# jweyn/DLWP-CS

Hardware: AMD Instinct MI355X
Metric: cubed-sphere samples/sec (fwd+bwd) (higher is better)
Workload: dtype bf16; 1 GPU; unet2 C48: x (32,6,48,48,14) per GPU, 14 out channels, base 32, MSE + Adam, fwd+bwd+update, bf16 activations + bf16 MFMA, fp32 master weights / gradients / Adam; global_batch=32, parallelism=dp1, hip_graphs=True

## Files before the change

dlwp-cs_amd/DLWP/_native.py:

```python
import ctypes
import os
import threading

import numpy as np
import torch

_HERE = os.path.dirname(os.path.abspath(__file__))
_TAG = os.environ.get('DLWPCS_LIB_TAG', '')
LIB_PATH = os.path.join(os.path.dirname(_HERE), 'lib', 'libdlwpcs%s.so' % ('_' + _TAG if _TAG else ''))

F32 = 0
BF16 = 1
I16 = 2
MAP_RENORMALIZE = 1
MSE_TARGET_F32 = 0x100
MSE_OVERWRITE = 0x200
ADAM_ZERO_GRAD = 1
HEAD_DEFER_STAGE2 = 2
LOSS_MSE, LOSS_MAE, LOSS_ACC = 0, 1, 2
REG_NONE, REG_MSE, REG_MAE, REG_GLOBAL = 0, 1, 2, 3
NORM_ALL, NORM_VALID = 0, 1
E_UNSUPPORTED = -2
ACT_NONE = 0
ACT_LEAKY_CLIP = 1
# ... 321 lines not shown
    'dlwpcs_state_repack': (c_int, [c_void_p, c_void_p, c_void_p, c_int, c_size_t, c_int, c_int, c_int, c_int, c_void_p]),
    'dlwpcs_head_mse_scratch_bytes': (c_size_t, []),
    'dlwpcs_head_mse_tail': (c_int, [c_void_p, c_float, c_int, c_void_p, c_void_p, c_void_p]),
    'dlwpcs_loss_tail_run': (c_int, [c_void_p, c_void_p]),
    'dlwpcs_head_mse_step': (c_int, [c_void_p, c_void_p, c_void_p, c_void_p, c_void_p, c_void_p, c_float, c_void_p, c_void_p,
                                     c_void_p, c_int, c_void_p, c_void_p]),
    'dlwpcs_head_mse_step_masked': (c_int, [c_void_p, c_void_p, c_void_p, c_void_p, c_void_p, c_void_p, c_float, c_void_p,
                                            c_void_p, c_void_p, c_int, c_void_p, c_float, c_float, c_void_p]),
    'dlwpcs_adam_step_dev': (c_int, [c_void_p, c_void_p, c_void_p, c_void_p, c_size_t, c_void_p, c_void_p, c_int,
                                     c_void_p]),
    'dlwpcs_batch_gather': (c_int, [c_void_p, ctypes.c_int64, c_int, ctypes.c_int64, c_void_p, c_int, c_void_p, c_int,
                                    c_int, c_int, c_int, c_void_p, c_int, c_int, c_int, c_int, c_int, c_void_p]),
    'dlwpcs_solar_fill': (c_int, [c_void_p, ctypes.c_int64, c_void_p, ctypes.c_int64, c_void_p, c_int, c_int, c_int, c_int,
                                  c_void_p, c_int, c_int, c_int, c_int, c_int, c_void_p]),
    'dlwpcs_channel_moments_scratch_bytes': (c_size_t, [c_void_p, ctypes.c_int64]),
    'dlwpcs_channel_moments': (c_int, [c_void_p, c_void_p, c_void_p, ctypes.c_int64, c_void_p, c_int, c_void_p, c_void_p, c_size_t,
                                       c_void_p]),
    'dlwpcs_channel_affine': (c_int, [c_void_p, c_void_p, c_void_p, c_void_p, c_int, c_void_p, c_void_p]),
    'dlwpcs_channel_range_scratch_bytes': (c_size_t, [ctypes.c_int64, ctypes.c_int64, ctypes.c_int64]),
    'dlwpcs_channel_range': (c_int, [c_void_p, ctypes.c_int64, ctypes.c_int64, ctypes.c_int64, c_void_p, c_void_p, c_void_p,
                                     c_size_t, c_void_p]),
    'dlwpcs_pack_i16': (c_int, [c_void_p, ctypes.c_int64, ctypes.c_int64, ctypes.c_int64, c_void_p, c_void_p, c_void_p, c_void_p]),
    'dlwpcs_unpack_i16': (c_int, [c_void_p, ctypes.c_int64, ctypes.c_int64, ctypes.c_int64, c_void_p, c_void_p, c_void_p,
                                  c_void_p]),
    'dlwpcs_batch_gather_i16': (c_int, [c_void_p, ctypes.c_int64, c_int, ctypes.c_int64, c_void_p, c_void_p, c_void_p, c_int,
                                        c_void_p, c_int, c_int, c_int, c_int, c_void_p, c_int, c_int, c_int, c_int, c_int,
                                        c_void_p]),
    'dlwpcs_comm_load': (c_int, [ctypes.c_char_p]),
    'dlwpcs_comm_unique_id': (c_int, [c_void_p]),
    'dlwpcs_comm_init': (c_int, [ctypes.POINTER(c_void_p), c_void_p, c_int, c_int]),
    'dlwpcs_comm_destroy': (c_int, [c_void_p]),
    'dlwpcs_allreduce_f32': (c_int, [c_void_p, c_void_p, c_size_t, c_void_p]),
    'dlwpcs_lds_oob_probe': (c_int, [c_void_p, c_void_p]),
    'dlwpcs_prof_enable': (c_int, [c_int]),
    'dlwpcs_prof_reset': (c_int, []),
    'dlwpcs_prof_count': (c_int, []),
    'dlwpcs_prof_get': (c_int, [c_int, ctypes.c_char_p, c_int, ctypes.POINTER(ctypes.c_double),
                                ctypes.POINTER(ctypes.c_double), ctypes.POINTER(ctypes.c_double)]),
    'dlwpcs_prof_known_tags': (c_int, []),
    'dlwpcs_prof_known_tag': (c_int, [c_int, ctypes.c_char_p, c_int]),
}

_lib = None
_lock = threading.Lock()


class NativeError(RuntimeError):
    pass


def lib():
    global _lib
    if _lib is None:
        with _lock:
            if _lib is None:
                if not os.path.exists(LIB_PATH):
                    raise NativeError(
                        'libdlwpcs.so not found at %s: build it with `python dlwp-cs_amd/build.py` '
                        '(or __graft_entry__.build()).  The DLWP-CS MI355X engine has no CPU fallback.' % LIB_PATH)
                handle = ctypes.CDLL(LIB_PATH)
                for name, (res, args) in PROTOTYPES.items():
                    fn = getattr(handle, name)
                    fn.restype = res
                    fn.argtypes = args
                _lib = handle
    return _lib
# ... 117 lines not shown
```

dlwp-cs_amd/csrc/conv_launch.h:

```cpp
#pragma once
#include "conv_ws.h"

namespace dlwpcs {

struct Work { double flops, bytes; };

static int tile_pixels(int BM, int No) {
    const int face_pix = No * No;
    int pix = BM < face_pix ? BM : face_pix;
    if (No <= BM) {
        int whole = (BM / No) * No;
        if (whole > face_pix) whole = face_pix;
        if (ceil_div(face_pix, whole) <= ceil_div(face_pix, pix)) pix = whole;
    }
    return pix;
}

static long ilv_cost(int pix, int face_pix, int B, int gx, int WM, int *gb, int *fb, bool split, int c2 = 2) {
    auto cost = [&](int npix) { const int mn = (npix + 31) / 32; return 4 * ceil_div(mn, WM) + c2; };
    const int nbl = ceil_div(face_pix, pix), cF = cost(pix), cL = cost(face_pix - (nbl - 1) * pix);
    const long ntiles = 6l * B * nbl;
    const long plain = (long)ceil_div((int)ntiles, gx) * cF;
    if (gb) *gb = 0;
    if (fb) *fb = 0;
    if (!split || cL >= cF || nbl < 2) return plain;
    const long F = 6l * (nbl - 1) * B, S = 6l * B;
    long best = plain;
    for (int GB = 1; GB < gx; ++GB) {
        const int GA = gx - GB;
        const long sB = ceil_div((int)S, GB) * (long)cL;
        for (long mB = 0; mB <= ceil_div((int)F, gx) + 1; ++mB) {
            const long FB = mB * GB < F ? mB * GB : F, FA = F - FB;
            const long cA = (long)ceil_div((int)FA, GA) * cF, cB = mB * cF + sB;
            const long mx = cA > cB ? cA : cB;
// ... 46 lines not shown
    P.magicNo = div_magic(P.No);
    P.magicN = div_magic(P.Nin);
    P.magicB = P.B > 1 ? div_magic(P.B) : 0;
    P.magicNblk = P.nblk_face > 1 ? div_magic(P.nblk_face) : 0;
    P.tile_rows_max = tile_rows_for(pix, P.Wt) + (KS - 1);
    P.ntiles = P.B * 6 * P.ncol * P.nblk_face;
    P.split_gb = P.split_fb = 0;
    P.tune = tune_bits();
    const size_t in_b = (size_t)P.tile_rows_max * P.W2 * (KC * ES + 16), w_b = (size_t)NTB * (KC / CGW) * (KS * KS + (EDGE ? 3 : 0)) * 1024;
    const bool rowpairs = (32 * MT) % (2 * P.Wt) == 0 && pix % (2 * P.Wt) == 0;
    const bool halfrows = !rowpairs && 32 * MT == P.Wt && WM == 4 && WN == 1 && pix == 4 * P.Wt && P.Wt % 4 == 0;
    bool pool = MODE != MODE_ZERO && P.pool_out != nullptr && P.No % 2 == 0 && P.Wt % 2 == 0 && (rowpairs || halfrows) &&
                strip_pix % pix == 0 && P.Cout % 32 == 0 && P.Cout % (16 / ES) == 0;
    if (EDGE) pool = pool && !MOUT && ES == 2 && P.dsplit > 0 && P.dsplit % 32 == 0;
    const size_t buf = in_b + w_b;
    size_t patch_b = (size_t)(WM * WN) * 32 * (32 * ES + 16);
    if (pool && 2 * buf + patch_b * MT <= 160 * 1024) patch_b *= MT; else pool = false;
    size_t lds = 2 * buf + patch_b;
    P.patches = 1;
    P.wstat = 0;
    const int nchunks = ceil_div(P.CG, KC / CGW);
    if (nchunks > 2 && nchunks <= 4 && (tune_bits() & TUNE_CONV_WSTAT) && 2 * in_b + nchunks * w_b + patch_b <= 160 * 1024) {
        P.wstat = nchunks;
        lds = 2 * in_b + nchunks * w_b + patch_b;
    } else if (lds > 160 * 1024) { lds = 2 * buf; P.patches = 0; pool = false; }
    if (!pool) P.pool_out = nullptr;
    {
        const bool head = P.head_w != nullptr && P.head_out != nullptr && ES == 2 && NT == 1 && WN == 1 && !EDGE && !MOUT && !MASK &&
                          MODE != MODE_ZERO && P.Cout == 32 && P.patches && !pool;
        if (head) P.out = P.head_out; else P.head_w = nullptr;
        if (P.head_done) *P.head_done = head ? 1 : 0;
    }
    P.colsplit = (pool && halfrows) ? 1 : 0;
    if (P.pool_done) *P.pool_done = pool ? 1 : 0;
    if ((MODE == MODE_ZERO || EDGE) && KS == 3 && P.patches && P.Cout % (16 / ES) == 0 && P.dsplit % (16 / ES) == 0) {
        if (P.direct_done) *P.direct_done = (P.d0 || P.d1) ? 1 : 0;
    } else {
        P.d0 = P.d1 = nullptr;
    }
    if (EDGE) {
        if (P.nblk_face < 2)
            return fail(DLWPCS_E_UNSUPPORTED, "conv: gather-form data gradient: a tile holds both edge rows of a face (N=%d)", P.No);
    }
    if (lds > 160 * 1024)
        return fail(DLWPCS_E_UNSUPPORTED, "conv: LDS tile of %zu bytes exceeds 160 KiB (face size %d)", lds, P.No);
    if (P.ncol > 1 && !P.patches)
        return fail(DLWPCS_E_UNSUPPORTED, "conv: internal: column strips need the line-store epilogue (face size %d)", P.No);
    if (P.tile_rows_max > 32)
        return fail(DLWPCS_E_UNSUPPORTED, "conv: %d tile rows exceed the producers' 5-bit row field", P.tile_rows_max);
    if ((size_t)P.tile_rows_max * P.W2 > (size_t)3 * NTHREADS)
        return fail(DLWPCS_E_UNSUPPORTED, "conv: tile of %d x %d pixels exceeds the producers' register capacity", P.tile_rows_max, P.W2);
    if ((long)6 * face_pix * P.Cout * ES >= (1l << 31))
        return fail(DLWPCS_E_UNSUPPORTED, "conv: one sample of the output (%ld bytes) exceeds the 32-bit store offsets",
                    (long)6 * face_pix * P.Cout * ES);
    if ((long)P.Nin * P.Nin * 6 >= (1l << 16) * 6 && (long)P.Nin * P.Nin >= (1l << 16))
        return fail(DLWPCS_E_UNSUPPORTED, "conv: face size %d too large for the 16-bit index arithmetic", P.Nin);
    auto kern = conv_mfma_ws_kernel<T, KS, KC, MT, NT, WM, WN, VW, MODE, MASK, TAIL8, MOUT, EDGE>;
    if (!MOUT || !(P.d0 || P.d1)) {
        if (!(P.d0)) P.m0 = nullptr;
        if (!(P.d1)) P.m1 = nullptr;
        if (!MOUT) P.m0 = P.m1 = nullptr;
    }
    if (P.mask_done) *P.mask_done = (MOUT && (P.m0 || P.m1)) ? ((P.m0 ? 1 : 0) | (P.m1 ? 2 : 0)) : 0;
    if (lds > 64 * 1024) {
        hipError_t e = hipFuncSetAttribute((const void *)kern, hipFuncAttributeMaxDynamicSharedMemorySize, (int)lds);
        if (e != hipSuccess) return fail(DLWPCS_E_LAUNCH, "conv: hipFuncSetAttribute: %s", hipGetErrorString(e));
// ... 64 lines not shown
```

dlwp-cs_amd/csrc/conv_small.hip:

```cpp
#include "conv_ws.h"

namespace dlwpcs {

struct SmallParams {
    const void *src;
    const void *wpk;
    const float *bias;
    const int32_t *table;
    void *out;
    void *d0;
    const void *m0;
    int B, Ns, No, W2;
    int Cin, Cout, CG, NT;
    int Q;
    uint32_t magicQ, magicW2, magicNo, magicNT, magicB;
    int act;
    float alpha, vmax;
    float m_alpha;
    uint32_t m_thr1;
    int patch_base;
};

constexpr int SM_THREADS = 256, SM_WAVES = 4;
constexpr int SM_PROW = 32 * 2 + 16;
constexpr int SM_U = 16;

template <bool BWD, int MTW>
__global__ void __launch_bounds__(SM_THREADS, 2) conv_small_kernel(const SmallParams P) {
    extern __shared__ __attribute__((aligned(16))) char smem[];
    const int tid = threadIdx.x;
    const int lane = tid & 63, wave = __builtin_amdgcn_readfirstlane(tid >> 6);
    const int half = lane >> 5, l31 = lane & 31;
    const uint32_t t = xcd_remap(blockIdx.x, gridDim.x);
    const int bf = P.magicNT ? __umulhi(t, P.magicNT) : (int)t;
    const int nt = (int)t - bf * P.NT;
    const int f = P.magicB ? __umulhi((uint32_t)bf, P.magicB) : bf;
    const int b = bf - f * P.B;
    const int v = f < 4 ? 0 : (f == 4 ? 1 : 2);
    const int RB = P.Cin * 2 + 16;
    const int face_pix = P.No * P.No;
    const int ncells = P.W2 * P.W2;
    const int nitems = ncells * P.Q;

    const uint4 *wsrc = reinterpret_cast<const uint4 *>(P.wpk) + ((size_t)v * P.NT + nt) * P.CG * 576 + lane;
    auto load_w = [&](int cg, uint4 (&w)[9]) __attribute__((always_inline)) {
        const uint4 *p = wsrc + (size_t)min(cg, P.CG - 1) * 576;
#pragma unroll
        for (int tap = 0; tap < 9; ++tap) w[tap] = p[tap * 64];
    };
    uint4 wa[9], wb[9];
    load_w(0, wa);

    {
        const int spix = 6 * P.Ns * P.Ns;
        const rsrc_t rs = make_rsrc(reinterpret_cast<const bf16_t *>(P.src) + (size_t)b * spix * P.Cin, (uint32_t)(spix * P.Cin * 2));
#pragma unroll 1
        for (int e0 = 0; e0 < nitems; e0 += SM_THREADS * SM_U) {
            int sp[SM_U];
#pragma unroll
            for (int u = 0; u < SM_U; ++u) {
                const int e = e0 + tid + u * SM_THREADS;
                const bool live = e < nitems;
                const int cell = __umulhi((uint32_t)e, P.magicQ);
                if constexpr (!BWD) {
                    sp[u] = P.table[live ? f * ncells + cell : 0];
                    if (!live) sp[u] = -1;
                } else {
                    const int ty = __umulhi((uint32_t)cell, P.magicW2), tx = cell - ty * P.W2;
                    const int vy = ty - 2, vx = tx - 2;
                    const bool ok = live & ((uint32_t)vy < (uint32_t)P.Ns) & ((uint32_t)vx < (uint32_t)P.Ns);
                    sp[u] = ok ? (f * P.Ns + vy) * P.Ns + vx : -1;
                }
            }
            u32x4 val[SM_U];
#pragma unroll
            for (int u = 0; u < SM_U; ++u) {
                const int e = e0 + tid + u * SM_THREADS;
                const int cell = __umulhi((uint32_t)e, P.magicQ), qv = e - cell * P.Q;
                const uint32_t off = sp[u] >= 0 ? (uint32_t)(sp[u] * P.Cin + qv * 8) * 2u : ST_SKIP;
                val[u] = __builtin_amdgcn_raw_buffer_load_b128(rs, off, 0, 0);
            }
#pragma unroll
            for (int u = 0; u < SM_U; ++u) {
                const int e = e0 + tid + u * SM_THREADS;
                const int cell = __umulhi((uint32_t)e, P.magicQ), qv = e - cell * P.Q;
                if (e < nitems) *reinterpret_cast<uint4 *>(smem + cell * RB + qv * 16) = make_uint4(val[u].x, val[u].y, val[u].z, val[u].w);
            }
        }
    }

    const int nmt = (face_pix + 31) >> 5;
    const int wv = (wave + (int)(blockIdx.x >> 3) + (int)(blockIdx.x >> 8)) & (SM_WAVES - 1);
    const int my_mt = max(0, min(MTW, (nmt - wv + SM_WAVES - 1) / SM_WAVES));
    int abase[MTW];
#pragma unroll
    for (int i = 0; i < MTW; ++i) {
        const int m = (wv + SM_WAVES * i) * 32 + l31;
        int base = 0;
        if (m < face_pix) {
            const int oy = __umulhi((uint32_t)m, P.magicNo), ox = m - oy * P.No;
            base = (oy * P.W2 + ox) * RB;
        }
        abase[i] = base + half * 16;
    }
    float4 bq[4];
#pragma unroll
    for (int jq = 0; jq < 4; ++jq)
        bq[jq] = P.bias ? *reinterpret_cast<const float4 *>(P.bias + (size_t)v * P.NT * 32 + nt * 32 + 8 * jq + 4 * half)
                        : make_float4(0.f, 0.f, 0.f, 0.f);
    f32x16 acc[MTW];

    load_w(1, wb);
    __syncthreads();
    if (my_mt == 0) return;

    auto matrix = [&](auto mta_tag) __attribute__((always_inline)) {
        constexpr int MTA = decltype(mta_tag)::value;
        constexpr int SM_R = MTA == 1 ? 6 : 3, SM_D = SM_R - 1;
        uint4 fa[SM_R][MTA];
#pragma unroll
        for (int i = 0; i < MTA; ++i)
#pragma unroll
            for (int jq = 0; jq < 4; ++jq) {
                acc[i][4 * jq] = bq[jq].x; acc[i][4 * jq + 1] = bq[jq].y; acc[i][4 * jq + 2] = bq[jq].z; acc[i][4 * jq + 3] = bq[jq].w;
            }
        auto rd = [&](int cg, int tap, uint4 (&a)[MTA]) __attribute__((always_inline)) {
            const char *lds = smem + cg * 32 + ((tap / 3) * P.W2 + tap % 3) * RB;
#pragma unroll
            for (int i = 0; i < MTA; ++i) a[i] = *reinterpret_cast<const uint4 *>(lds + abase[i]);
        };
#pragma unroll
        for (int st = 0; st < SM_D; ++st) rd(0, st, fa[st % SM_R]);
        __builtin_amdgcn_sched_group_barrier(0x100, SM_D * MTA, 0);
#pragma unroll 1
        for (int cg = 0; cg < P.CG; cg += 2) {
#pragma unroll
            for (int st = 0; st < 18; ++st) {
                rd(cg + (st + SM_D) / 9, (st + SM_D) % 9, fa[(st + SM_D) % SM_R]);
#pragma unroll
                for (int i = 0; i < MTA; ++i) frag_mma<bf16_t>(acc[i], st < 9 ? wa[st] : wb[st - 9], fa[st % SM_R][i]);
                __builtin_amdgcn_sched_group_barrier(0x100, MTA, 0);
                __builtin_amdgcn_sched_group_barrier(0x008, MTA, 0);
                if (st == 8) { asm volatile("" ::: "memory"); load_w(cg + 2, wa); }
                if (st == 17) { asm volatile("" ::: "memory"); load_w(cg + 3, wb); }
            }
        }
    };
    if (MTW >= 3 && my_mt >= 3) matrix(std::integral_constant<int, (MTW >= 3 ? 3 : 1)>{});
    else if (MTW >= 2 && my_mt == 2) matrix(std::integral_constant<int, (MTW >= 2 ? 2 : 1)>{});
    else matrix(std::integral_constant<int, 1>{});

    constexpr int NPS = 2;
    uint32_t soff[MTW][NPS];
    uint32_t ssel = 0;
    const int c = nt * 32 + (lane & 3) * 8;
#pragma unroll
    for (int i = 0; i < MTW; ++i)
#pragma unroll
        for (int ps = 0; ps < NPS; ++ps) {
            const int m = (wv + SM_WAVES * i) * 32 + ps * 16 + (lane >> 2);
// ... 96 lines not shown
        if (lds > 64 * 1024) {
            hipError_t e = hipFuncSetAttribute((const void *)kern, hipFuncAttributeMaxDynamicSharedMemorySize, (int)lds);
            if (e != hipSuccess) return fail(DLWPCS_E_LAUNCH, "conv_small: hipFuncSetAttribute: %s", hipGetErrorString(e));
        }
        hipLaunchKernelGGL(kern, dim3(grid), dim3(SM_THREADS), lds, s, P);
        return check_launch("conv_small");
    };
    if (mtw == 1) return go(conv_small_kernel<BWD, 1>);
    if (mtw == 2) return go(conv_small_kernel<BWD, 2>);
    return go(conv_small_kernel<BWD, 3>);
}

int launch_conv_small(const ConvKParams &K, hipStream_t s) {
    const bool bwd = K.mode == MODE_ZERO;
    if (K.mode != MODE_HALO && !bwd) return fail(DLWPCS_E_UNSUPPORTED, "conv_small: serves halo convolutions and their data gradients");
    const int N = K.Nin;
    if (K.C1 != 0 || K.up0 || K.ymask || K.pool_out || K.head_w || K.edge)
        return fail(DLWPCS_E_UNSUPPORTED, "conv_small: one source, no upsampling, no mask on load, no pooled or folded second output");
    if (K.No != (bwd ? N + 2 : N) || !conv_small_serves(K.B, N, K.Cin, K.Cout))
        return fail(DLWPCS_E_UNSUPPORTED, "conv_small: N=%d Cin=%d Cout=%d outside faces of <= 320 cells with channel counts that are multiples of 32",
                    N, K.Cin, K.Cout);
    if (bwd && K.d1) return fail(DLWPCS_E_UNSUPPORTED, "conv_small: one source");
    if (bwd && K.d0 && K.dsplit != K.Cout) return fail(DLWPCS_E_UNSUPPORTED, "conv_small: one source");
    SmallParams P{};
    P.src = K.src0; P.wpk = K.wpk; P.bias = K.bias; P.table = K.table; P.out = K.out;
    P.d0 = bwd ? K.d0 : nullptr;
    P.m0 = (bwd && K.d0) ? K.m0 : nullptr;
    P.B = K.B; P.Ns = N; P.No = K.No; P.W2 = K.No + 2;
    P.Cin = K.Cin; P.Cout = K.Cout; P.CG = K.Cin / 16; P.NT = K.Cout / 32; P.Q = K.Cin / 8;
    P.magicQ = div_magic(P.Q); P.magicW2 = div_magic(P.W2); P.magicNo = div_magic(P.No);
    P.magicNT = P.NT > 1 ? div_magic(P.NT) : 0; P.magicB = P.B > 1 ? div_magic(P.B) : 0;
    P.act = K.act; P.alpha = K.alpha; P.vmax = K.vmax;
    P.m_alpha = K.m_alpha; P.m_thr1 = K.m_thr1;
    const size_t in_b = (size_t)P.W2 * P.W2 * (P.Cin * 2 + 16);
    P.patch_base = (int)in_b;
    const size_t lds = in_b + (size_t)SM_WAVES * 32 * SM_PROW;
    const int nmt = ceil_div(P.No * P.No, 32), mtw = ceil_div(nmt, SM_WAVES);
    const long nwg = (long)P.B * 6 * P.NT;
    if (lds > 160 * 1024 || mtw > 3 || nwg >= (1l << 16) || P.W2 * P.W2 * P.Q >= (1 << 16))
        return fail(DLWPCS_E_UNSUPPORTED, "conv_small: B=%d N=%d Cin=%d beyond the kernel's LDS tile or index range", P.B, N, P.Cin);
    if (K.direct_done) *K.direct_done = (bwd && P.d0) ? 1 : 0;
    if (K.mask_done) *K.mask_done = P.m0 ? 1 : 0;
    if (K.pool_done) *K.pool_done = 0;
    if (K.head_done) *K.head_done = 0;
    if (K.dry_run || K.B == 0) return DLWPCS_OK;
    return bwd ? launch_small_t<true>(P, mtw, lds, (unsigned)nwg, s) : launch_small_t<false>(P, mtw, lds, (unsigned)nwg, s);
}

}
```

dlwp-cs_amd/csrc/conv_ws.h:

```cpp
#pragma once
#include <stdlib.h>
#include <type_traits>
#include "common.h"
#include "mfma_common.h"

namespace dlwpcs {

enum { MODE_DIRECT = 0, MODE_HALO = 1, MODE_ZERO = 2 };

struct ConvKParams {
    const void *src0, *src1;
    const void *ymask;
    const void *wpk;
    const float *bias;
    void *out;
    const int32_t *table;
    int edge;
    int B, Nin, No;
    int C0, C1, Cin, Cout;
    int CG, NTtot;
    int up0;
    int mode;
    int act;
    float alpha, vmax;
    int pix_per_block;
    int nblk_face;
    int W2;
    uint32_t magicW2, magicNo, magicN;
    uint32_t magicB, magicNblk;
    int patches;
    int wstat;
    void *d0, *d1;
    int dsplit;
    const void *m0, *m1;
    float m_alpha, m_vmax;
    uint32_t m_thr1;
    int *direct_done;
    int *mask_done;
    int dry_run;
    void *pool_out;
    int *pool_done;
    const void *pool_mask;
    int colsplit;
    const void *head_w;
    const float *head_b;
    void *head_out;
    int *head_done;
    int tune;
    int tile_rows_max;
    int ntiles;
    int split_gb, split_fb;
    int Wt, ncol;
    uint32_t magicWt, magicNcol;
    int ilv_fwd;
};

struct ConvEdgeArgs { const int32_t *src; int8_t wids[36]; };

enum { TUNE_WG_PRODUCER_PRIO = 1, TUNE_CONV_PRODUCER_PRIO = 2, TUNE_CONV_WEIGHTS_STAY = 4, TUNE_CONV_SPLIT_N = 16,
       TUNE_CONV_SPLIT2_BWD = 32, TUNE_CONV_WSTAT = 64, TUNE_CONV_STAGGER = 256, TUNE_CONV_ILV = 512, TUNE_CONV_STRIPS = 1024,
       TUNE_CONV_ILV_FWD = 2048 };
static int tune_bits() {
    static int v = -1;
    if (v < 0) { const char *e = getenv("DLWPCS_TUNE"); v = e ? atoi(e) : (TUNE_WG_PRODUCER_PRIO | TUNE_CONV_PRODUCER_PRIO | TUNE_CONV_WEIGHTS_STAY | TUNE_CONV_SPLIT_N | TUNE_CONV_SPLIT2_BWD | TUNE_CONV_WSTAT |
                               TUNE_CONV_STAGGER | TUNE_CONV_ILV | TUNE_CONV_STRIPS | TUNE_CONV_ILV_FWD | (3 << 12));
                 }
    return v;
}

template <typename T, int KS, int KC, int MT, int NT, int WM, int WN, int VW, int MODE, bool MASK, bool TAIL8 = false, bool MOUT = false,
          bool EDGE = false>
__device__ __forceinline__ void conv_ws_body(const ConvKParams &P, char *smem, const uint32_t lw, const int G, const int by,
                                             const ConvEdgeArgs &E = ConvEdgeArgs{}) {
    static_assert(!TAIL8 || (VW == 8 && sizeof(T) == 2 && !MASK), "TAIL8: bf16 16-B vectors, forward only");
    static_assert(!MOUT || ((MODE == MODE_ZERO || EDGE) && KS == 3 && sizeof(T) == 2 && !MASK), "MOUT: bf16 data gradient, direct mode");
    static_assert(!EDGE || (MODE == MODE_HALO && KS == 3 && !MASK && !TAIL8 && VW * sizeof(T) == 16), "EDGE: gather-form data gradient");
    constexpr int ES = sizeof(T);
    constexpr int CGW = 32 / ES;
    constexpr int TAPS = KS * KS;
    constexpr int RB = KC * ES + 16;
    constexpr int KCG = KC / CGW;
    constexpr int Q = KC / VW;
    constexpr int NTB = NT * WN;
    constexpr int NCT = 64 * WM * WN;
    constexpr int GF4 = TAPS * 64;
    constexpr int WF4M = NTB * KCG * TAPS * 64;
    constexpr int XF4 = NTB * KCG * 64;
    constexpr int WF4 = EDGE ? WF4M + 3 * XF4 : WF4M;
    constexpr int ITS = 3 * KC / VW;
    using OkMask = typename std::conditional<(ITS > 32), uint64_t, uint32_t>::type;
    static_assert(ITS <= 64, "one validity bit per input vector");
    constexpr int ITW = (WF4 + NCT - 1) / NCT;
    static_assert(NCT % Q == 0, "thread -> channel-vector mapping must not depend on the item");
    static_assert(KC % CGW == 0 && KC % VW == 0, "chunk must hold whole operand groups and whole vectors");
    typedef typename VecT<T, VW>::type V;
    const int in_bytes = P.tile_rows_max * P.W2 * RB;
    const int in_step = P.wstat ? in_bytes : in_bytes + WF4 * 16;
    const int w_base = P.wstat ? 2 * in_bytes : in_bytes;
    const int w_step = P.wstat ? WF4 * 16 : in_bytes + WF4 * 16;
    const int patch_base = P.wstat ? 2 * in_bytes + P.wstat * WF4 * 16 : 2 * (in_bytes + WF4 * 16);

    const int tid = threadIdx.x;
    const bool is_producer = tid >= NCT;
    const int nt0 = by * NTB;
    const int face_pix = P.No * P.No;
    const int strip_pix = P.No * P.Wt;
    const int g0 = P.up0 ? (P.Nin >> 1) : P.Nin;
    const int nchunks = (P.CG + KCG - 1) / KCG;

    constexpr bool ILV_OK = (MODE == MODE_ZERO || (MODE == MODE_HALO && !EDGE && KS == 3)) && MT == 3 && sizeof(T) == 4;
    const bool ilv = ILV_OK && (P.tune & TUNE_CONV_ILV) != 0 && (MODE == MODE_ZERO || P.ilv_fwd != 0);
    const int nbl = P.nblk_face;
    const bool csplit = ilv && P.split_gb > 0;
    int t_first = 0, t_last = 0;
    int f0 = 0, f1 = 0, s0 = 0, s1 = 0;
    if (csplit) {
        const int GB = P.split_gb, GA = G - GB;
        const int Ftot = 6 * (nbl - 1) * P.B, Stot = 6 * P.B, FA = Ftot - P.split_fb;
        if ((int)lw < GA) {
            f0 = (int)(((long)FA * lw) / GA); f1 = (int)(((long)FA * (lw + 1)) / GA);
        } else {
            const int u = (int)lw - GA;
            f0 = FA + (int)(((long)P.split_fb * u) / GB); f1 = FA + (int)(((long)P.split_fb * (u + 1)) / GB);
            s0 = (int)(((long)Stot * u) / GB); s1 = (int)(((long)Stot * (u + 1)) / GB);
        }
    } else {
        t_first = (int)(((long)P.ntiles * lw) / G);
        t_last = (int)(((long)P.ntiles * (lw + 1)) / G);
    }
// ... 130 lines not shown
                if (idx < WF4) reinterpret_cast<uint4 *>(wa)[idx] = wv[u];
            }
        };
        auto issue = [&](const Geo &gc, int ch, V (&val)[ITS], V (&ymv)[MASK ? ITS : 1], OkMask &okm) __attribute__((always_inline)) {
            const int wkey = (EDGE ? gc.fcls : gc.v) * 1024 + ch;
            const int area = P.wstat ? ch : (g & 1);
            const bool need_w = !(P.tune & TUNE_CONV_WEIGHTS_STAY) || wres[area] != wkey;
            wres[area] = wkey;
            if (need_w) {
                uint4 wv[ITW];
                load_w(gc.v, gc.fcls, ch, wv);
                store_w(area, wv);
            }
            const T *sb; int cstride, cs_ld, sh; bool c_ok, up;
            chunk_src(gc, ch, sb, cstride, cs_ld, sh, c_ok, up);
            const T *ymb = MASK ? reinterpret_cast<const T *>(P.ymask) + (size_t)gc.b * 6 * g0 * g0 * P.C0 : nullptr;
            okm = 0;
#pragma unroll
            for (int i = 0; i < ITS; ++i) {
                int idx = sidx[i];
                if constexpr (SUP) idx += up ? sup[i] : 0;
                const bool ok = c_ok && idx >= 0;
                int pix = ok ? idx : 0;
                if constexpr (!SUP) pix = up ? upmap(pix) : pix;
                const size_t oo = ok ? (size_t)pix * cstride + cs_ld : 0;
                if constexpr (TAIL8) val[i] = *reinterpret_cast<const uint4_a4 *>(sb + oo);
                else val[i] = *reinterpret_cast<const V *>(sb + oo);
                if (MASK) ymv[i] = *reinterpret_cast<const V *>(ymb + oo);
                okm |= (OkMask)ok << i;
            }
        };
        auto commit = [&](const Geo &gc, int ch, V (&val)[ITS], V (&ymv)[MASK ? ITS : 1], OkMask okm) __attribute__((always_inline)) {
            char *buf = smem + (g & 1) * in_step;
            if constexpr (TAIL8) {
                const T *sb; int cstride, cs_ld, sh; bool c_ok, up;
                chunk_src(gc, ch, sb, cstride, cs_ld, sh, c_ok, up);
                if (sh) {
#pragma unroll
                    for (int i = 0; i < ITS; ++i) val[i] = vshl_dwords(val[i], sh);
                }
            }
            if (MASK) {
#pragma unroll
                for (int i = 0; i < ITS; ++i) vmask(val[i], ymv[i], P.alpha, P.vmax);
            }
#pragma unroll
            for (int i = 0; i < ITS; ++i) {
                const int e = ptid + i * NCT;
                if (e < gc.nitems) *reinterpret_cast<V *>(buf + (e / Q) * RB + qv * ES) = vsel(((okm >> i) & 1u) != 0, val[i]);
            }
            __syncthreads();
            ++g;
        };

        int cur_combo = -1;
        V val[ITS], ymv[MASK ? ITS : 1];
        OkMask okm = 0;
        for (int q = 0; q < n_my; ++q) {
            const Geo gq = geo_of(tile_of(q));
            if (gq.combo != cur_combo) { lookup(gq); cur_combo = gq.combo; }
            for (int ch = 0; ch < nchunks; ++ch) {
                issue(gq, ch, val, ymv, okm);
                commit(gq, ch, val, ymv, okm);
            }
        }
        if (P.tune & TUNE_CONV_PRODUCER_PRIO) __builtin_amdgcn_s_setprio(0);
        return;
    }

    const int lane = tid & 63, wave = __builtin_amdgcn_readfirstlane(tid >> 6);
    const int wm = wave / WN, wn = wave % WN;
    const int half = lane >> 5, l31 = lane & 31;

    auto tile_pix = [&](int loc) __attribute__((always_inline)) {
        const int lin = ilv ? (((loc >> 5) * WM + wm) * 32 + (loc & 31)) : wm * MT * 32 + loc;
        const int hN = P.Wt >> 1;
        const int r = loc >= hN ? 1 : 0;
        const int cs = (2 * (wm >> 1) + r) * P.Wt + (wm & 1) * hN + (loc - r * hN);
        return P.colsplit ? cs : lin;
    };
    f32x16 acc[MT][NT];
    constexpr int LPP = 32 * ES / 16;
// ... 43 lines not shown
    const int pool_cs = EDGE ? P.dsplit : P.Cout;
    auto pools_nt = [&](int nt) { return !EDGE || (nt0 + wn * NT + nt) * 32 < P.dsplit; };
    char *const patch0 = smem + patch_base + wave * (32 * PROW) * (pooling ? MT : 1);
    const int patch_step = pooling ? 32 * PROW : 0;
    constexpr int PITEMS = MT * 8 * LPP;
    constexpr int PNP = (PITEMS + 63) / 64;
    uint32_t plds0[PNP], plds1[PNP], pgo[NT][PNP];
    auto pool_setup = [&](const Geo &gq) {
        const int hN = P.No >> 1;
        const int Wl = P.colsplit ? (P.Wt >> 1) : P.Wt, hW = Wl >> 1;
#pragma unroll
        for (int ps = 0; ps < PNP; ++ps) {
            const int item = ps * 64 + lane;
            const int pp = min(item / LPP, MT * 8 - 1), q = item % LPP;
            const int prow = pp / hW, pcol = pp - prow * hW;
            const int i00 = 2 * prow * Wl + 2 * pcol, i10 = i00 + Wl;
            plds0[ps] = (uint32_t)((i00 >> 5) * (32 * PROW) + (i00 & 31) * PROW + q * 16);
            plds1[ps] = (uint32_t)((i10 >> 5) * (32 * PROW) + (i10 & 31) * PROW + q * 16);
            const int gm = gq.m0 + tile_pix(i00);
            const int oy = __umulhi((uint32_t)gm, P.magicWt), ox = gq.x0 + (gm - oy * P.Wt);
#pragma unroll
            for (int nt = 0; nt < NT; ++nt) {
                const int c = (nt0 + wn * NT + nt) * 32 + q * (16 / ES);
                const bool ok = item / LPP < MT * 8 && tile_pix(i00) < gq.npix && c < pool_cs;
                pgo[nt][ps] = ok ? (uint32_t)((((gq.f * hN + (oy >> 1)) * hN + (ox >> 1)) * pool_cs + c) * ES) : ST_SKIP;
            }
        }
    };
    auto setup = [&](const Geo &gq) {
        if (gq.combo != cur_combo) {
            cur_combo = gq.combo;
#pragma unroll
            for (int mt = 0; mt < MT; ++mt) {
                const int m = tile_pix(mt * 32 + l31);
                int base = 0;
                if (m < gq.npix) {
                    const int gm = gq.m0 + m;
                    const int oy = __umulhi((uint32_t)gm, P.magicWt);
                    const int ox = gm - oy * P.Wt;
                    base = ((oy - gq.y0) * P.W2 + ox) * RB;
                }
                abase[mt] = base + half * 16;
            }
            if constexpr (EDGE) {
                const int ylast = __umulhi((uint32_t)(gq.m0 + gq.npix - 1), P.magicNo);
                const bool maybe = gq.f >= 4 || gq.y0 == 0 || ylast == P.No - 1;
                bool any = false, two = false;
#pragma unroll
                for (int w = 0; w < (MT + 3) / 4; ++w) ewp[w] = 0;
#pragma unroll
                for (int mt = 0; mt < MT; ++mt) {
                    const int m = tile_pix(mt * 32 + l31);
                    const int gm = gq.m0 + min(m, gq.npix - 1);
                    const int oy = __umulhi((uint32_t)gm, P.magicNo), ox = gm - oy * P.No;
                    const bool border = maybe && m < gq.npix && ((oy == 0) | (oy == P.No - 1) | (ox == 0) | (ox == P.No - 1));
                    const int ord = oy == 0 ? ox : (oy == P.No - 1 ? P.No + ox : 2 * P.No + 2 * (oy - 1) + (ox ? 1 : 0));
                    int4 e0 = make_int4(-1, -1, -1, -1), e1 = make_int4(-1, -1, 0, 0);
                    if (maybe) {
                        const int4 *esrc = reinterpret_cast<const int4 *>(E.src + ((size_t)gq.f * (4 * P.No - 4) + (border ? ord : 0)) * 8);
                        e0 = esrc[0]; e1 = esrc[1];
                    }
                    auto fld = [&](int pos) {
                        const int pa = (max(pos, 0) * 11) >> 5, pb = max(pos, 0) - 3 * pa;
                        return (border && pos >= 0) ? (uint32_t)(abase[mt] + (pa * P.W2 + pb) * RB) >> 4 : 0x8000u;
                    };
                    es[mt][0] = fld(e0.x) | fld(e0.y) << 16;
                    es[mt][1] = fld(e0.z) | fld(e0.w) << 16;
                    es[mt][2] = fld(e1.x) | fld(e1.y) << 16;
                    const uint32_t wrong = border ? (uint32_t)e1.z : 0u;
                    ewp[mt / 4] |= ((wrong & 15u) | ((wrong >> 5) << 4)) << (8 * (mt % 4));
                    any |= border && (wrong != 0 || e0.x >= 0 || e0.y >= 0 || e0.z >= 0 || e0.w >= 0 || e1.x >= 0 || e1.y >= 0);
                    two |= border && (e0.w >= 0 || e1.x >= 0 || e1.y >= 0);
                }
                e_any = __builtin_amdgcn_ballot_w64(any) != 0 ? 1u : 0u;
                e_two = __builtin_amdgcn_ballot_w64(two) != 0 ? 1u : 0u;
#pragma unroll
                for (int mt = 0; mt < MT; ++mt) asm volatile("" : "+v"(es[mt][0]), "+v"(es[mt][1]), "+v"(es[mt][2]));
#pragma unroll
                for (int w = 0; w < (MT + 3) / 4; ++w) asm volatile("" : "+v"(ewp[w]));
            }
            if constexpr (MODE != MODE_ZERO) {
                if (pooling) pool_setup(gq);
            }
            if constexpr (SOFF) {
                ssel = 0;
#pragma unroll
                for (int nt = 0; nt < NT; ++nt)
#pragma unroll
                    for (int mt = 0; mt < MT; ++mt)
#pragma unroll
                        for (int ps = 0; ps < NPS; ++ps) {
                            uint32_t sel;
                            soff[nt][mt][ps] = store_off(gq, nt, mt, ps, sel);
                            ssel |= sel << (2 * ((nt * MT + mt) * NPS + ps));
                        }
            }
        }
// ... 287 lines not shown
                T *dst = outp + (size_t)(gq.m0 + m) * P.Cout + cot + 4 * half;
#pragma unroll
                for (int jq = 0; jq < 4; ++jq) {
                    const int co = cot + 8 * jq + 4 * half;
                    const float4 v4 = quad(std::integral_constant<int, 0>{}, acc[mt][nt], jq);
                    if (m >= gq.npix) continue;
                    if (wide) {
                        if (co < P.Cout) {
                            if constexpr (ES == 4) *reinterpret_cast<float4 *>(dst + 8 * jq) = v4;
                            else *reinterpret_cast<uint2 *>(dst + 8 * jq) = make_uint2(f2bf2(v4.x, v4.y), f2bf2(v4.z, v4.w));
                        }
                    } else {
                        const float vs[4] = {v4.x, v4.y, v4.z, v4.w};
#pragma unroll
                        for (int u = 0; u < 4; ++u)
                            if (co + u < P.Cout) {
                                if constexpr (ES == 4) dst[8 * jq + u] = vs[u];
                                else dst[8 * jq + u] = f2bf(vs[u]);
                            }
                    }
                }
            }
        }
    };

    constexpr int NSTEP = KCG * TAPS;
    auto mma_chunk = [&](int ch, auto mta_tag) {
        constexpr int MTA = decltype(mta_tag)::value;
        const char *lds_in = smem + (g & 1) * in_step, *lds_w = smem + w_base + (P.wstat ? ch : (g & 1)) * w_step;
        uint4 fa[2][MT], fb[2][NT];
        auto load_frag = [&](int step, uint4 (&a)[MT], uint4 (&bw)[NT]) {
            const int cgl = step / TAPS, tap = step % TAPS;
            const int dy = tap / KS, dx = tap % KS;
            const int tapoff = (dy * P.W2 + dx) * RB + cgl * 32;
#pragma unroll
            for (int mt = 0; mt < MTA; ++mt) a[mt] = *reinterpret_cast<const uint4 *>(lds_in + abase[mt] + tapoff);
#pragma unroll
            for (int nt = 0; nt < NT; ++nt)
                bw[nt] = *reinterpret_cast<const uint4 *>(
                    lds_w + ((((wn * NT + nt) * KCG + cgl) * TAPS + tap) * 2 + half) * 512 + l31 * 16);
        };
        load_frag(0, fa[0], fb[0]);
        __builtin_amdgcn_sched_group_barrier(0x100, MTA + NT, 0);
#pragma unroll
        for (int step = 0; step < NSTEP; ++step) {
            const int cur = step & 1;
            if (step + 1 < NSTEP) load_frag(step + 1, fa[cur ^ 1], fb[cur ^ 1]);
#pragma unroll
            for (int mt = 0; mt < MTA; ++mt)
#pragma unroll
                for (int nt = 0; nt < NT; ++nt) frag_mma<T>(acc[mt][nt], fb[cur][nt], fa[cur][mt]);
            __builtin_amdgcn_sched_group_barrier(0x100, MTA + NT, 0);
            __builtin_amdgcn_sched_group_barrier(0x008, MmaPerFrag<T>::N * MTA * NT, 0);
        }
    };

    auto mma_chunk_edge = [&](const Geo &gq, int ch, auto two_tag) {
      if constexpr (EDGE) {
        constexpr int NSETS = decltype(two_tag)::value ? 2 : 1;
        constexpr int NX = NSETS * 3 * KCG;
        const char *lds_in = smem + (g & 1) * in_step, *lds_w = smem + w_base + (P.wstat ? ch : (g & 1)) * w_step;
        const char *lds_x = lds_w + WF4M * 16;
        uint32_t (&rs)[MT][3] = es;
        uint32_t (&rw)[(MT + 3) / 4] = ewp;
#pragma unroll
        for (int mt = 0; mt < MT; ++mt) asm volatile("" : "+v"(rs[mt][0]), "+v"(rs[mt][1]), "+v"(rs[mt][2]));
#pragma unroll
        for (int w = 0; w < (MT + 3) / 4; ++w) asm volatile("" : "+v"(rw[w]));
        uint4 fa[2][MT], fb[2][NT];
        auto load_frag = [&](int step, uint4 (&a)[MT], uint4 (&bw)[NT]) {
            if (step < NSTEP) {
                const int cgl = step / TAPS, tap = step % TAPS;
                const int dy = tap / KS, dx = tap % KS;
                const int tapoff = (dy * P.W2 + dx) * RB + cgl * 32;
#pragma unroll
                for (int mt = 0; mt < MT; ++mt) {
                    int base = abase[mt];
                    if (tap != TAPS / 2) base += (int)((rw[mt / 4] >> (8 * (mt % 4) + (tap < TAPS / 2 ? tap : tap - 1))) & 1u) << 23;
                    a[mt] = *reinterpret_cast<const uint4 *>(lds_in + base + tapoff);
                }
#pragma unroll
                for (int nt = 0; nt < NT; ++nt)
                    bw[nt] = *reinterpret_cast<const uint4 *>(
                        lds_w + ((((wn * NT + nt) * KCG + cgl) * TAPS + tap) * 2 + half) * 512 + l31 * 16);
            } else {
                const int x = step - NSTEP, j = x / KCG, cgl = x % KCG;
#pragma unroll
                for (int mt = 0; mt < MT; ++mt) {
                    const uint32_t f16 = (j & 1) ? rs[mt][j >> 1] >> 16 : rs[mt][j >> 1] & 0xffffu;
                    a[mt] = *reinterpret_cast<const uint4 *>(lds_in + (int)(f16 << 4) + cgl * 32);
                }
#pragma unroll
                for (int nt = 0; nt < NT; ++nt)
                    bw[nt] = *reinterpret_cast<const uint4 *>(
                        lds_x + (((j % 3) * NTB * KCG + (wn * NT + nt) * KCG + cgl) * 2 + half) * 512 + l31 * 16);
            }
        };
        load_frag(0, fa[0], fb[0]);
        __builtin_amdgcn_sched_group_barrier(0x100, MT + NT, 0);
#pragma unroll
        for (int step = 0; step < NSTEP + NX; ++step) {
            const int cur = step & 1;
            if (step + 1 < NSTEP + NX) load_frag(step + 1, fa[cur ^ 1], fb[cur ^ 1]);
#pragma unroll
            for (int mt = 0; mt < MT; ++mt)
#pragma unroll
                for (int nt = 0; nt < NT; ++nt) frag_mma<T>(acc[mt][nt], fb[cur][nt], fa[cur][mt]);
// ... 58 lines not shown
```

include/dlwpcs.h:

```cpp
#ifndef DLWPCS_H
#define DLWPCS_H

#include <stddef.h>
#include <stdint.h>

#ifdef __cplusplus
extern "C" {
#endif

#define DLWPCS_VERSION 105

#define DLWPCS_OK             0
#define DLWPCS_E_INVALID     -1
#define DLWPCS_E_UNSUPPORTED -2
#define DLWPCS_E_WORKSPACE   -3
#define DLWPCS_E_LAUNCH      -4

#define DLWPCS_F32  0
#define DLWPCS_BF16 1

#define DLWPCS_ACT_NONE        0
#define DLWPCS_ACT_LEAKY_CLIP  1

typedef void *dlwpcs_stream_t;
// ... 578 lines not shown
#define DLWPCS_AFFINE_MAX_CHANNELS 1024
typedef struct dlwpcs_chan_desc {
    int64_t R, C, S;
    int64_t row_stride, chan_stride, inner_stride;
    int64_t dst_row_stride, dst_chan_stride, dst_inner_stride;
} dlwpcs_chan_desc;
size_t dlwpcs_channel_moments_scratch_bytes(const dlwpcs_chan_desc *d, int64_t n_rows);
int dlwpcs_channel_moments(const dlwpcs_chan_desc *d, const float *src, const int32_t *rows, int64_t n_rows,
                           const double *center, int skipna, double *out, void *scratch, size_t scratch_bytes,
                           dlwpcs_stream_t stream);
int dlwpcs_channel_affine(const dlwpcs_chan_desc *d, const float *src, const float *a, const float *b, int mode, float *dst,
                          dlwpcs_stream_t stream);

size_t dlwpcs_channel_range_scratch_bytes(int64_t T, int64_t V, int64_t S);
int dlwpcs_channel_range(const float *src, int64_t T, int64_t V, int64_t S, float *range, int64_t *nonfinite, void *scratch,
                         size_t scratch_bytes, dlwpcs_stream_t stream);
int dlwpcs_pack_i16(const float *src, int64_t T, int64_t V, int64_t S, const float *scale, const float *offset, int16_t *dst,
                    dlwpcs_stream_t stream);
int dlwpcs_unpack_i16(const int16_t *src, int64_t T, int64_t V, int64_t S, const float *scale, const float *offset, float *dst,
                      dlwpcs_stream_t stream);
int dlwpcs_batch_gather_i16(const int16_t *array, int64_t T, int V, int64_t S, const float *scale, const float *offset,
                            const int32_t *samples_dev, int B, const int32_t *var_idx_dev, int nv, int n_steps, int t_off,
                            int t_stride, void *out, int Ctot, int c_off, int c_stride, int channels_last, int dtype,
                            dlwpcs_stream_t stream);

int dlwpcs_comm_load(const char *librccl_path);
int dlwpcs_comm_unique_id(void *id128);
int dlwpcs_comm_init(void **comm, const void *id128, int rank, int world);
int dlwpcs_comm_destroy(void *comm);
int dlwpcs_allreduce_f32(void *comm, float *buf, size_t n, dlwpcs_stream_t stream);

int dlwpcs_lds_oob_probe(int32_t *nonzero_dev, dlwpcs_stream_t stream);

int dlwpcs_prof_enable(int on);
int dlwpcs_prof_reset(void);
int dlwpcs_prof_count(void);
int dlwpcs_prof_get(int i, char *tag, int tag_len, double *ms, double *flops, double *bytes);
int dlwpcs_prof_known_tags(void);
int dlwpcs_prof_known_tag(int i, char *tag, int tag_len);

#ifdef __cplusplus
}
#endif
#endif
```

Measured before the change: 49610 samples/s.

## Pad LDS input tile rows to reduce bank conflicts in conv fragment reads

Adds a per-row byte padding (row_bytes) to the LDS input tile layout in the main conv kernel and the small-face kernel, choosing the pad with a host-side model of LDS bank conflicts for the MFMA A-fragment reads. Producers, address bases, tap offsets and edge gather offsets all switch to the row_bytes stride. Padding is rejected if it overflows LDS or, for the small kernel, lowers occupancy. It is on by default for the main conv and behind an off-by-default bit for the small kernel, and a diagnostic query entry point is exported.

Result: no change. 49250 samples/s (-0.7%).

```diff
diff --git a/dlwp-cs_amd/DLWP/_native.py b/dlwp-cs_amd/DLWP/_native.py
--- a/dlwp-cs_amd/DLWP/_native.py
+++ b/dlwp-cs_amd/DLWP/_native.py
@@ -377,6 +377,7 @@
     'dlwpcs_comm_destroy': (c_int, [c_void_p]),
     'dlwpcs_allreduce_f32': (c_int, [c_void_p, c_void_p, c_size_t, c_void_p]),
     'dlwpcs_lds_oob_probe': (c_int, [c_void_p, c_void_p]),
+    'dlwpcs_conv_rowpad_info': (c_int, [c_int, c_int, c_int, c_int, c_int, c_int, ctypes.c_int64, c_int, c_void_p]),
     'dlwpcs_prof_enable': (c_int, [c_int]),
     'dlwpcs_prof_reset': (c_int, []),
     'dlwpcs_prof_count': (c_int, []),
diff --git a/dlwp-cs_amd/csrc/conv_launch.h b/dlwp-cs_amd/csrc/conv_launch.h
--- a/dlwp-cs_amd/csrc/conv_launch.h
+++ b/dlwp-cs_amd/csrc/conv_launch.h
@@ -1,5 +1,6 @@
 #pragma once
 #include "conv_ws.h"
+#include "lds_banks.h"
 
 namespace dlwpcs {
 
@@ -112,6 +113,12 @@
         if (P.head_done) *P.head_done = head ? 1 : 0;
     }
     P.colsplit = (pool && halfrows) ? 1 : 0;
+    {
+        constexpr int RB = KC * ES + 16;
+        const int pad = (VW * ES == 16 && (tune_bits() & TUNE_CONV_ROWPAD)) ? lds_row_pad_fit(lds_row_pad(P.Wt, P.W2, RB, pix, !P.colsplit), 2 * P.tile_rows_max, lds, false) : 0;
+        P.row_bytes = P.W2 * RB + pad;
+        lds += (size_t)2 * P.tile_rows_max * pad;
+    }
     if (P.pool_done) *P.pool_done = pool ? 1 : 0;
     if ((MODE == MODE_ZERO || EDGE) && KS == 3 && P.patches && P.Cout % (16 / ES) == 0 && P.dsplit % (16 / ES) == 0) {
         if (P.direct_done) *P.direct_done = (P.d0 || P.d1) ? 1 : 0;
diff --git a/dlwp-cs_amd/csrc/conv_small.hip b/dlwp-cs_amd/csrc/conv_small.hip
--- a/dlwp-cs_amd/csrc/conv_small.hip
+++ b/dlwp-cs_amd/csrc/conv_small.hip
@@ -1,4 +1,5 @@
 #include "conv_ws.h"
+#include "lds_banks.h"
 
 namespace dlwpcs {
 
@@ -19,6 +20,7 @@
     float m_alpha;
     uint32_t m_thr1;
     int patch_base;
+    int row_bytes;
 };
 
 constexpr int SM_THREADS = 256, SM_WAVES = 4;
@@ -41,6 +43,7 @@
     const int face_pix = P.No * P.No;
     const int ncells = P.W2 * P.W2;
     const int nitems = ncells * P.Q;
+    const int rpad = P.row_bytes - P.W2 * RB;
 
     const uint4 *wsrc = reinterpret_cast<const uint4 *>(P.wpk) + ((size_t)v * P.NT + nt) * P.CG * 576 + lane;
     auto load_w = [&](int cg, uint4 (&w)[9]) __attribute__((always_inline)) {
@@ -84,7 +87,9 @@
             for (int u = 0; u < SM_U; ++u) {
                 const int e = e0 + tid + u * SM_THREADS;
                 const int cell = __umulhi((uint32_t)e, P.magicQ), qv = e - cell * P.Q;
-                if (e < nitems) *reinterpret_cast<uint4 *>(smem + cell * RB + qv * 16) = make_uint4(val[u].x, val[u].y, val[u].z, val[u].w);
+                int at = cell * RB + qv * 16;
+                if (rpad) at += (int)__umulhi((uint32_t)cell, P.magicW2) * rpad;
+                if (e < nitems) *reinterpret_cast<uint4 *>(smem + at) = make_uint4(val[u].x, val[u].y, val[u].z, val[u].w);
             }
         }
     }
@@ -95,13 +100,9 @@
     int abase[MTW];
 #pragma unroll
     for (int i = 0; i < MTW; ++i) {
-        const int m = (wv + SM_WAVES * i) * 32 + l31;
-        int base = 0;
-        if (m < face_pix) {
-            const int oy = __umulhi((uint32_t)m, P.magicNo), ox = m - oy * P.No;
-            base = (oy * P.W2 + ox) * RB;
-        }
-        abase[i] = base + half * 16;
+        const int m = min((wv + SM_WAVES * i) * 32 + l31, face_pix - 1);
+        const int oy = __umulhi((uint32_t)m, P.magicNo), ox = m - oy * P.No;
+        abase[i] = oy * P.row_bytes + ox * RB + half * 16;
     }
     float4 bq[4];
 #pragma unroll
@@ -125,7 +126,7 @@
                 acc[i][4 * jq] = bq[jq].x; acc[i][4 * jq + 1] = bq[jq].y; acc[i][4 * jq + 2] = bq[jq].z; acc[i][4 * jq + 3] = bq[jq].w;
             }
         auto rd = [&](int cg, int tap, uint4 (&a)[MTA]) __attribute__((always_inline)) {
-            const char *lds = smem + cg * 32 + ((tap / 3) * P.W2 + tap % 3) * RB;
+            const char *lds = smem + cg * 32 + (tap / 3) * P.row_bytes + (tap % 3) * RB;
 #pragma unroll
             for (int i = 0; i < MTA; ++i) a[i] = *reinterpret_cast<const uint4 *>(lds + abase[i]);
         };
@@ -288,7 +289,11 @@
     P.magicNT = P.NT > 1 ? div_magic(P.NT) : 0; P.magicB = P.B > 1 ? div_magic(P.B) : 0;
     P.act = K.act; P.alpha = K.alpha; P.vmax = K.vmax;
     P.m_alpha = K.m_alpha; P.m_thr1 = K.m_thr1;
-    const size_t in_b = (size_t)P.W2 * P.W2 * (P.Cin * 2 + 16);
+    const int RB = P.Cin * 2 + 16;
+    const size_t lds0 = (size_t)P.W2 * P.W2 * RB + (size_t)SM_WAVES * 32 * SM_PROW;
+    const int pad = (tune_bits() & TUNE_CONV_ROWPAD_SMALL) ? lds_row_pad_fit(lds_row_pad(P.No, P.W2, RB, P.No * P.No), P.W2, lds0, true) : 0;
+    P.row_bytes = P.W2 * RB + pad;
+    const size_t in_b = (size_t)P.W2 * P.row_bytes;
     P.patch_base = (int)in_b;
     const size_t lds = in_b + (size_t)SM_WAVES * 32 * SM_PROW;
     const int nmt = ceil_div(P.No * P.No, 32), mtw = ceil_div(nmt, SM_WAVES);
@@ -304,3 +309,18 @@
 }
 
 }
+
+extern "C" int dlwpcs_conv_rowpad_info(int wt, int w2, int rb, int tile_pix, int pad, int rows, int64_t lds_bytes, int per_cu, int32_t info[8]) {
+    using namespace dlwpcs;
+    if (!info) return fail(DLWPCS_E_INVALID, "conv_rowpad_info: null info");
+    if (wt < 1 || w2 < wt || rb < 16 || rb % 16 || tile_pix < 1 || pad < 0 || pad % 16 || rows < 0 || lds_bytes < 1)
+        return fail(DLWPCS_E_INVALID, "conv_rowpad_info: wt=%d w2=%d rb=%d tile_pix=%d pad=%d rows=%d: not a tile geometry", wt, w2, rb, tile_pix, pad, rows);
+    auto milli = [&](int p) { return (int32_t)(lds_frag_cycles(wt, w2, rb, tile_pix, p) * 1000.0 + 0.5); };
+    const int want = lds_row_pad(wt, w2, rb, tile_pix);
+    int why = 0;
+    const int got = lds_row_pad_fit(want, rows, (size_t)lds_bytes, per_cu != 0, &why);
+    info[0] = milli(pad); info[1] = want; info[2] = milli(want); info[3] = got; info[4] = why;
+    info[5] = (int32_t)(lds_bytes + (int64_t)rows * got);
+    info[6] = (tune_bits() & (per_cu ? TUNE_CONV_ROWPAD_SMALL : TUNE_CONV_ROWPAD)) ? 1 : 0; info[7] = 0;
+    return DLWPCS_OK;
+}
diff --git a/dlwp-cs_amd/csrc/conv_ws.h b/dlwp-cs_amd/csrc/conv_ws.h
--- a/dlwp-cs_amd/csrc/conv_ws.h
+++ b/dlwp-cs_amd/csrc/conv_ws.h
@@ -26,6 +26,7 @@
     int pix_per_block;
     int nblk_face;
     int W2;
+    int row_bytes;
     uint32_t magicW2, magicNo, magicN;
     uint32_t magicB, magicNblk;
     int patches;
@@ -59,11 +60,11 @@
 
 enum { TUNE_WG_PRODUCER_PRIO = 1, TUNE_CONV_PRODUCER_PRIO = 2, TUNE_CONV_WEIGHTS_STAY = 4, TUNE_CONV_SPLIT_N = 16,
        TUNE_CONV_SPLIT2_BWD = 32, TUNE_CONV_WSTAT = 64, TUNE_CONV_STAGGER = 256, TUNE_CONV_ILV = 512, TUNE_CONV_STRIPS = 1024,
-       TUNE_CONV_ILV_FWD = 2048 };
+       TUNE_CONV_ILV_FWD = 2048, TUNE_CONV_ROWPAD = 1 << 18, TUNE_CONV_ROWPAD_SMALL = 1 << 19 };
 static int tune_bits() {
     static int v = -1;
     if (v < 0) { const char *e = getenv("DLWPCS_TUNE"); v = e ? atoi(e) : (TUNE_WG_PRODUCER_PRIO | TUNE_CONV_PRODUCER_PRIO | TUNE_CONV_WEIGHTS_STAY | TUNE_CONV_SPLIT_N | TUNE_CONV_SPLIT2_BWD | TUNE_CONV_WSTAT |
-                               TUNE_CONV_STAGGER | TUNE_CONV_ILV | TUNE_CONV_STRIPS | TUNE_CONV_ILV_FWD | (3 << 12));
+                               TUNE_CONV_STAGGER | TUNE_CONV_ILV | TUNE_CONV_STRIPS | TUNE_CONV_ILV_FWD | TUNE_CONV_ROWPAD | (3 << 12));
                  }
     return v;
 }
@@ -94,7 +95,7 @@
     static_assert(NCT % Q == 0, "thread -> channel-vector mapping must not depend on the item");
     static_assert(KC % CGW == 0 && KC % VW == 0, "chunk must hold whole operand groups and whole vectors");
     typedef typename VecT<T, VW>::type V;
-    const int in_bytes = P.tile_rows_max * P.W2 * RB;
+    const int in_bytes = P.tile_rows_max * P.row_bytes;
     const int in_step = P.wstat ? in_bytes : in_bytes + WF4 * 16;
     const int w_base = P.wstat ? 2 * in_bytes : in_bytes;
     const int w_step = P.wstat ? WF4 * 16 : in_bytes + WF4 * 16;
@@ -291,6 +292,7 @@
         };
         auto commit = [&](const Geo &gc, int ch, V (&val)[ITS], V (&ymv)[MASK ? ITS : 1], OkMask okm) __attribute__((always_inline)) {
             char *buf = smem + (g & 1) * in_step;
+            const int rpad = P.row_bytes - P.W2 * RB;
             if constexpr (TAIL8) {
                 const T *sb; int cstride, cs_ld, sh; bool c_ok, up;
                 chunk_src(gc, ch, sb, cstride, cs_ld, sh, c_ok, up);
@@ -306,7 +308,8 @@
 #pragma unroll
             for (int i = 0; i < ITS; ++i) {
                 const int e = ptid + i * NCT;
-                if (e < gc.nitems) *reinterpret_cast<V *>(buf + (e / Q) * RB + qv * ES) = vsel(((okm >> i) & 1u) != 0, val[i]);
+                const int rowpad = VW * ES == 16 ? (slot_c[i] & 31) * rpad : 0;
+                if (e < gc.nitems) *reinterpret_cast<V *>(buf + (e / Q) * RB + rowpad + qv * ES) = vsel(((okm >> i) & 1u) != 0, val[i]);
             }
             __syncthreads();
             ++g;
@@ -416,15 +419,10 @@
             cur_combo = gq.combo;
 #pragma unroll
             for (int mt = 0; mt < MT; ++mt) {
-                const int m = tile_pix(mt * 32 + l31);
-                int base = 0;
-                if (m < gq.npix) {
-                    const int gm = gq.m0 + m;
-                    const int oy = __umulhi((uint32_t)gm, P.magicWt);
-                    const int ox = gm - oy * P.Wt;
-                    base = ((oy - gq.y0) * P.W2 + ox) * RB;
-                }
-                abase[mt] = base + half * 16;
+                const int gm = gq.m0 + min(tile_pix(mt * 32 + l31), gq.npix - 1);
+                const int oy = __umulhi((uint32_t)gm, P.magicWt);
+                const int ox = gm - oy * P.Wt;
+                abase[mt] = (oy - gq.y0) * P.row_bytes + ox * RB + half * 16;
             }
             if constexpr (EDGE) {
                 const int ylast = __umulhi((uint32_t)(gq.m0 + gq.npix - 1), P.magicNo);
@@ -446,7 +444,7 @@
                     }
                     auto fld = [&](int pos) {
                         const int pa = (max(pos, 0) * 11) >> 5, pb = max(pos, 0) - 3 * pa;
-                        return (border && pos >= 0) ? (uint32_t)(abase[mt] + (pa * P.W2 + pb) * RB) >> 4 : 0x8000u;
+                        return (border && pos >= 0) ? (uint32_t)(abase[mt] + pa * P.row_bytes + pb * RB) >> 4 : 0x8000u;
                     };
                     es[mt][0] = fld(e0.x) | fld(e0.y) << 16;
                     es[mt][1] = fld(e0.z) | fld(e0.w) << 16;
@@ -800,7 +798,7 @@
         auto load_frag = [&](int step, uint4 (&a)[MT], uint4 (&bw)[NT]) {
             const int cgl = step / TAPS, tap = step % TAPS;
             const int dy = tap / KS, dx = tap % KS;
-            const int tapoff = (dy * P.W2 + dx) * RB + cgl * 32;
+            const int tapoff = dy * P.row_bytes + dx * RB + cgl * 32;
 #pragma unroll
             for (int mt = 0; mt < MTA; ++mt) a[mt] = *reinterpret_cast<const uint4 *>(lds_in + abase[mt] + tapoff);
 #pragma unroll
@@ -840,7 +838,7 @@
             if (step < NSTEP) {
                 const int cgl = step / TAPS, tap = step % TAPS;
                 const int dy = tap / KS, dx = tap % KS;
-                const int tapoff = (dy * P.W2 + dx) * RB + cgl * 32;
+                const int tapoff = dy * P.row_bytes + dx * RB + cgl * 32;
 #pragma unroll
                 for (int mt = 0; mt < MT; ++mt) {
                     int base = abase[mt];
diff --git a/dlwp-cs_amd/csrc/lds_banks.h b/dlwp-cs_amd/csrc/lds_banks.h
--- /dev/null
+++ b/dlwp-cs_amd/csrc/lds_banks.h
@@ -0,0 +1,62 @@
+#pragma once
+#include <stddef.h>
+#include <stdint.h>
+
+namespace dlwpcs {
+
+static inline double lds_frag_cycles(int Wt, int W2, int RB, int pix, int pad) {
+    static const int8_t grp[2][16] = {{0, 1, 2, 3, 12, 13, 14, 15, 20, 21, 22, 23, 24, 25, 26, 27},
+                                      {4, 5, 6, 7, 8, 9, 10, 11, 16, 17, 18, 19, 28, 29, 30, 31}};
+    if (Wt < 1 || pix < 1) return 1.0;
+    const int row_bytes = W2 * RB + pad, nmt = (pix + 31) / 32;
+    long total = 0;
+    for (int j = 0; j < nmt; ++j)
+        for (int s = 0; s < 2; ++s) {
+            int addr[16], na = 0, cnt[16] = {0}, worst = 1;
+            for (int k = 0; k < 16; ++k) {
+                int m = j * 32 + grp[s][k];
+                if (m > pix - 1) m = pix - 1;
+                const int a = (m / Wt) * row_bytes + (m % Wt) * RB;
+                bool seen = false;
+                for (int u = 0; u < na; ++u) seen |= addr[u] == a;
+                if (seen) continue;
+                addr[na++] = a;
+                const int c = ++cnt[(a >> 4) & 15];
+                if (c > worst) worst = c;
+            }
+            total += worst;
+        }
+    return (double)total / (2 * nmt);
+}
+
+static inline int lds_row_pad(int Wt, int W2, int RB, int pix, bool consecutive = true) {
+    if (!consecutive) return 0;
+    struct Key { int Wt, W2, RB, pix, pad; };
+    static thread_local Key memo[8] = {};
+    static thread_local int next = 0;
+    for (const Key &k : memo)
+        if (k.Wt == Wt && k.W2 == W2 && k.RB == RB && k.pix == pix) return k.pad;
+    double best = lds_frag_cycles(Wt, W2, RB, pix, 0);
+    int pad = 0;
+    for (int p = 16; p < 256 && best > 1.0; p += 16) {
+        const double c = lds_frag_cycles(Wt, W2, RB, pix, p);
+        if (c < best) { best = c; pad = p; }
+    }
+    memo[next] = Key{Wt, W2, RB, pix, pad};
+    next = (next + 1) & 7;
+    return pad;
+}
+
+static inline int lds_row_pad_fit(int pad, int rows, size_t lds0, bool per_cu, int *why = nullptr) {
+    constexpr size_t LDS_CU = 160 * 1024;
+    int w = 0;
+    if (pad > 0) {
+        const size_t lds1 = lds0 + (size_t)rows * pad;
+        if (lds1 > LDS_CU) w = 2;
+        else if (per_cu && LDS_CU / lds1 < LDS_CU / lds0) w = 1;
+    }
+    if (why) *why = w;
+    return w ? 0 : pad;
+}
+
+}
diff --git a/include/dlwpcs.h b/include/dlwpcs.h
--- a/include/dlwpcs.h
+++ b/include/dlwpcs.h
@@ -634,6 +634,9 @@
 
 int dlwpcs_lds_oob_probe(int32_t *nonzero_dev, dlwpcs_stream_t stream);
 
+int dlwpcs_conv_rowpad_info(int wt, int w2, int rb, int tile_pix, int pad, int rows, int64_t lds_bytes, int per_cu,
+                            int32_t info[8]);
+
 int dlwpcs_prof_enable(int on);
 int dlwpcs_prof_reset(void);
 int dlwpcs_prof_count(void);
```
